# cmeraki/audiotoken

Hardware: AMD Instinct MI355X
Metric: audio-sec tokenized / wall-sec (acoustic + semantic_m) (higher is better)
Workload: dtype f32 (linear layers: two fp16 pieces per operand, three MFMA products, fp32 accumulate)

## Files before the change

### audiotoken_amd/_cabi.py

```python
from __future__ import annotations

import ctypes as C
import os
from pathlib import Path

import numpy as np

_LIB_PATH = Path(__file__).resolve().parent / "lib" / "libaudiotoken_hip.so"
_lib = None


class HipLibraryError(RuntimeError):
    pass


class SegmentDesc(C.Structure):
    _fields_ = [("pcm", C.c_void_p), ("table", C.c_void_p), ("chunk_off", C.c_int64), ("chunk_len", C.c_int32), ("out_start", C.c_int32),
                ("valid_len", C.c_int32), ("fmt", C.c_int32), ("scale", C.c_float), ("o", C.c_int32), ("n", C.c_int32), ("width", C.c_int32),
                ("chunk_out_len", C.c_int32)]


PCM_S16, PCM_S32, PCM_F32, PCM_U8 = 0, 1, 2, 3


# ... 114 lines not shown
    "at_hubert_profile_read": (C.c_int, [C.c_void_p, C.c_char_p, C.c_size_t, C.POINTER(C.c_float), C.POINTER(C.c_int), C.c_int]),
    "at_encodec_range_sites": (C.c_int, [C.c_char_p, C.c_size_t]),
    "at_encodec_range_report": (C.c_int, [C.c_void_p, C.POINTER(C.c_float), C.c_int]),
    "at_w2vbert_range_sites": (C.c_int, [C.c_char_p, C.c_size_t]),
    "at_w2vbert_range_report": (C.c_int, [C.c_void_p, C.POINTER(C.c_float), C.c_int]),
    "at_w2vbert_site_scales": (C.c_int, [C.c_void_p, C.POINTER(C.c_float), C.c_int]),
    "at_hubert_site_scales": (C.c_int, [C.c_void_p, C.POINTER(C.c_float), C.c_int]),
    "at_w2vbert_layer_status": (C.c_int, [C.c_void_p, C.POINTER(C.c_int32), C.c_int]),
    "at_hubert_layer_status": (C.c_int, [C.c_void_p, C.POINTER(C.c_int32), C.c_int]),
    "at_hubert_range_sites": (C.c_int, [C.c_char_p, C.c_size_t]),
    "at_hubert_range_report": (C.c_int, [C.c_void_p, C.POINTER(C.c_float), C.c_int]),
    "at_segments_from_pcm": (C.c_int, [C.c_void_p, C.c_int, C.c_int, C.c_float, C.c_void_p, C.c_void_p, C.c_void_p]),
    "at_clock_stamp": (C.c_int, [C.c_void_p, C.c_void_p]),
    "at_resample_rows": (C.c_int, [C.c_void_p, C.c_int, C.c_void_p, C.c_void_p]),
    "at_resample_rows_check": (C.c_int, [C.c_void_p, C.c_int]),
    "at_segments_zmuv_workspace_bytes": (C.c_size_t, [C.c_int, C.c_int]),
    "at_segments_from_pcm_zmuv": (C.c_int, [C.c_void_p, C.c_int, C.c_int, C.c_int, C.c_float, C.c_float, C.c_void_p, C.c_void_p, C.c_void_p, C.c_size_t, C.c_void_p]),
    "at_pcm_peaks": (C.c_int, [C.c_void_p, C.c_void_p, C.c_int, C.c_int64, C.c_void_p, C.c_void_p]),
    "at_pcm_pack": (C.c_int, [C.c_void_p, C.c_void_p, C.c_int, C.c_int64, C.c_float, C.c_void_p, C.c_void_p, C.c_void_p]),
    "at_flac_encode_workspace_bytes": (C.c_size_t, [C.c_int]),
    "at_flac_encode_rows": (C.c_int, [C.c_void_p, C.c_void_p, C.c_int, C.c_int, C.c_float, C.c_void_p, C.c_void_p, C.c_int64, C.c_void_p, C.c_void_p, C.c_size_t,
                                      C.c_void_p]),
    "at_flac_encode_pcm16": (C.c_int64, [C.c_void_p, C.c_int64, C.c_int, C.c_void_p, C.c_int64, C.c_void_p, C.c_int64, C.c_int64]),
    "at_flac_write_frames": (C.c_int64, [C.c_void_p, C.c_int, C.c_void_p, C.c_int64, C.c_int, C.c_void_p, C.c_int, C.c_void_p, C.c_int64, C.c_void_p]),
    "at_flac_streaminfo": (C.c_int, [C.c_int, C.c_int, C.c_int, C.c_int, C.c_int, C.c_int64, C.c_void_p]),
    "at_flac_info": (C.c_int, [C.c_void_p, C.c_size_t, C.POINTER(C.c_int), C.POINTER(C.c_int), C.POINTER(C.c_int), C.POINTER(C.c_int64), C.c_void_p]),
    "at_flac_decode": (C.c_int64, [C.c_void_p, C.c_size_t, C.c_void_p, C.c_int64]),
    "at_op_layernorm": (C.c_int, [C.c_void_p, C.c_void_p, C.c_void_p, C.c_void_p, C.c_void_p, C.c_int64, C.c_int, C.c_void_p]),
    "at_op_relpos_attention": (C.c_int, [C.c_void_p, C.c_void_p, C.c_void_p, C.c_void_p, C.c_int, C.c_int, C.c_void_p]),
    "at_op_relpos_attention_kvp": (C.c_int, [C.c_void_p, C.c_void_p, C.c_void_p, C.c_float, C.c_void_p, C.c_int, C.c_int, C.c_int, C.c_int, C.c_void_p, C.c_size_t,
                                             C.c_void_p, C.c_void_p]),
    "at_op_dwconv_ln_swish": (C.c_int, [C.c_void_p, C.c_void_p, C.c_void_p, C.c_void_p, C.c_void_p, C.c_int, C.c_int, C.c_void_p]),
    "at_op_dwconv_stream": (C.c_int, [C.c_void_p, C.c_void_p, C.c_void_p, C.c_void_p, C.c_void_p, C.c_int, C.c_int, C.c_void_p]),
    "at_op_vq_argmax": (C.c_int, [C.c_void_p, C.c_void_p, C.c_void_p, C.c_void_p, C.c_int64, C.c_int, C.c_int, C.c_void_p]),
    "at_op_vq_argmax_refined": (C.c_int, [C.c_void_p, C.c_void_p, C.c_void_p, C.c_void_p, C.c_void_p, C.c_int64, C.c_int, C.c_int, C.c_void_p]),
    "at_kmeans_device_bytes": (C.c_size_t, [C.c_int64, C.c_int, C.c_int]),
    "at_kmeans_create": (C.c_void_p, [C.c_int, C.c_int64, C.c_int, C.c_int]),
    "at_kmeans_destroy": (None, [C.c_void_p]),
    "at_kmeans_set_option": (C.c_int, [C.c_void_p, C.c_char_p, C.c_int]),
    "at_kmeans_get_option": (C.c_int, [C.c_void_p, C.c_char_p]),
    "at_kmeans_set_data": (C.c_int, [C.c_void_p, C.c_void_p, C.c_float, C.c_void_p]),
    "at_kmeans_plusplus": (C.c_int, [C.c_void_p, C.c_void_p, C.c_int, C.c_void_p, C.c_void_p, C.c_void_p]),
    "at_kmeans_assign": (C.c_int, [C.c_void_p, C.c_void_p, C.c_float, C.c_void_p, C.c_void_p, C.c_void_p]),
    "at_kmeans_update": (C.c_int, [C.c_void_p, C.c_void_p, C.c_void_p, C.c_void_p, C.c_void_p, C.c_void_p, C.c_void_p, C.c_void_p]),
    "at_kmeans_layernorm": (C.c_int, [C.c_void_p, C.c_void_p, C.c_int64, C.c_int, C.c_int, C.c_void_p, C.c_size_t, C.c_void_p]),
    "at_kmeans_row_d2": (C.c_int, [C.c_void_p, C.c_void_p, C.c_void_p]),
    "at_kmeans_relocations": (C.c_int, [C.c_void_p, C.c_void_p, C.c_void_p]),
    "at_op_gemm": (C.c_int, [C.POINTER(GemmDesc), C.c_void_p]),
    "at_op_gemm_dual": (C.c_int, [C.POINTER(GemmDesc), C.c_void_p, C.c_int64, C.c_int, C.c_int, C.c_void_p]),
    "at_op_gemm_route": (C.c_int, [C.POINTER(GemmDesc), C.c_void_p, C.c_int64, C.c_int, C.c_int, C.POINTER(C.c_int32)]),
    "at_op_attention_f32": (C.c_int, [C.c_void_p, C.c_void_p, C.c_void_p, C.c_void_p, C.c_int, C.c_int, C.c_int, C.c_void_p]),
    "at_required_tensors": (C.c_int, [C.c_char_p, C.c_int, C.c_int, C.c_char_p, C.c_size_t]),
    "at_op_gemm_split": (C.c_int, [C.c_void_p, C.c_void_p, C.c_void_p, C.c_void_p, C.c_int, C.c_int, C.c_int, C.c_int, C.c_float, C.c_int,
                                   C.c_void_p, C.c_size_t, C.c_void_p, C.c_void_p]),
    "at_op_conv_split": (C.c_int, [C.c_void_p, C.c_void_p, C.c_void_p, C.c_void_p, C.c_int, C.c_int, C.c_int, C.c_int, C.c_int, C.c_int, C.c_float,
                                  C.c_void_p, C.c_size_t, C.c_void_p, C.c_void_p]),
    "at_op_rvq_encode_split": (C.c_int, [C.c_void_p, C.c_int64, C.c_int, C.c_void_p, C.c_void_p, C.c_int, C.c_void_p, C.c_int, C.c_float,
                                        C.c_void_p, C.c_size_t, C.c_void_p, C.c_void_p]),
    "at_op_rvq_encode": (C.c_int, [C.c_void_p, C.c_int64, C.c_int, C.c_void_p, C.c_void_p, C.c_int, C.c_void_p, C.c_void_p]),
    "at_gpt_create": (C.c_void_p, [C.c_int]),
    "at_gpt_set_tensor": (C.c_int, [C.c_void_p, C.c_char_p, C.c_void_p, C.POINTER(C.c_int64), C.c_int]),
    "at_gpt_finalize": (C.c_int, [C.c_void_p]),
    "at_gpt_destroy": (None, [C.c_void_p]),
    "at_gpt_num_layers": (C.c_int, [C.c_void_p]),
    "at_gpt_vocab": (C.c_int, [C.c_void_p]),
    "at_gpt_block_size": (C.c_int, [C.c_void_p]),
# ... 186 lines not shown
```

### audiotoken_amd/csrc/dwconv_stream.hip

```cpp
#include "at_common.h"
#include "w2vbert_kernels.h"
#include "split_scheme.h"

#include <type_traits>

namespace at {

namespace {

constexpr int DS_K = 31;
constexpr int DS_RB = 8;
constexpr int DS_WIN = DS_RB + DS_K - 1;
constexpr int DS_C = 1024;

__device__ __forceinline__ float ds_quad_xor1(float x) { return __builtin_bit_cast(float, __builtin_amdgcn_mov_dpp(__builtin_bit_cast(int, x), 0xB1, 0xF, 0xF, true)); }
__device__ __forceinline__ float ds_quad_xor2(float x) { return __builtin_bit_cast(float, __builtin_amdgcn_mov_dpp(__builtin_bit_cast(int, x), 0x4E, 0xF, 0xF, true)); }

template <bool SECOND>
__device__ __forceinline__ void ds_reduce(float (&v)[DS_RB], float (*sq)[256], float (*stat)[4], int c, int lane) {
#pragma unroll
    for (int i = 0; i < DS_RB; ++i) {
        float p = v[i] + ds_quad_xor1(v[i]);
        p = p + ds_quad_xor2(p);
        if ((lane & 3) == 0) sq[i][c >> 2] = p;
    }
    __syncthreads();
    const int wave = c >> 6;
    if (wave < DS_RB) {
        float t[4];
#pragma unroll
        for (int grp = 0; grp < 4; ++grp) t[grp] = sq[wave][grp * 64 + lane];
#pragma unroll
        for (int off = 32; off >= 1; off >>= 1)
#pragma unroll
            for (int grp = 0; grp < 4; ++grp) t[grp] += __shfl_xor(t[grp], off);
        if (lane == 0) {
            const float total = (t[0] + t[1]) + (t[2] + t[3]);
            if (!SECOND) {
                stat[wave][0] = total * (1.0f / 1024.0f);
            } else {
                const float vr = total * (1.0f / 1024.0f);
                const float rstd = 1.0f / sqrtf(vr + 1e-5f);
                stat[wave][1] = rstd;
                stat[wave][2] = -rstd * stat[wave][0];
            }
        }
    }
    __syncthreads();
}

}

template <class SC>
__global__ __launch_bounds__(1024, 1) void dwconv_stream_kernel(const float* __restrict__ g, const float* __restrict__ w ,
                                                                const float* __restrict__ gamma, const float* __restrict__ beta,
                                                                float* __restrict__ out, int T, int seg_len, void* __restrict__ pieces, long long rows_pad,
                                                                float scale, int* __restrict__ status) {
    __shared__ float sq[DS_RB][256];
    __shared__ __attribute__((aligned(16))) float stat[DS_RB][4];
    __shared__ __attribute__((aligned(16))) float otile[DS_RB][DS_C + 4];
    const int c = threadIdx.x, lane = c & 63;
    const int b = blockIdx.y;
    const int t_begin = blockIdx.x * seg_len;
    if (t_begin >= T) return;
    const int t_end = t_begin + seg_len < T ? t_begin + seg_len : T;
    const long long base = (long long)b * T;
    const float* gc = g + base * DS_C + c;

    float wt[DS_K];
#pragma unroll
    for (int j = 0; j < DS_K; ++j) wt[j] = w[j * DS_C + c];
    float xw[DS_WIN];
#pragma unroll
    for (int k = 0; k < DS_K - 1; ++k) {
        const int t = t_begin - (DS_K - 1) + k;
        xw[k] = t >= 0 ? gc[(long long)t * DS_C] : 0.f;
    }
    float pre[DS_RB];
    auto prefetch = [&](int tb) {
#pragma unroll
        for (int i = 0; i < DS_RB; ++i) {
            int t = tb + i;
            t = t < T ? t : T - 1;
            pre[i] = gc[(long long)t * DS_C];
        }
    };
    prefetch(t_begin);
    RangeMax over;
    (void)over;
    for (int tb = t_begin; tb < t_end; tb += DS_RB) {
#pragma unroll
        for (int i = 0; i < DS_RB; ++i) xw[DS_K - 1 + i] = pre[i];
        if (tb + DS_RB < t_end) prefetch(tb + DS_RB);
        float acc[DS_RB];
#pragma unroll
        for (int i = 0; i < DS_RB; ++i) {
            float a = 0.f;
#pragma unroll
            for (int tap = 0; tap < DS_K; ++tap) a = __builtin_fmaf(wt[tap], xw[i + tap], a);
            acc[i] = a;
        }
        float term[DS_RB];
#pragma unroll
        for (int i = 0; i < DS_RB; ++i) term[i] = acc[i];
        ds_reduce<false>(term, sq, stat, c, lane);
#pragma unroll
        for (int i = 0; i < DS_RB; ++i) {
            const float d = acc[i] - stat[i][0];
            const float m = __fmul_rn(d, d);
            const float f = __builtin_fmaf(d, d, ds_quad_xor1(m));
            term[i] = (lane & 1) ? 0.f : f;
        }
        ds_reduce<true>(term, sq, stat, c, lane);
        const float* gp = gamma;
        const float* bp = beta;
        asm volatile("" : "+s"(gp), "+s"(bp));
        const float gm = gp[c], bt = bp[c];
#pragma unroll
        for (int i = 0; i < DS_RB; ++i) {
            const int t = tb + i;
            const float o = swishf_(fmaf(fmaf(acc[i], stat[i][1], stat[i][2]), gm, bt));
            if constexpr (std::is_void<SC>::value) {
                if (t < t_end) out[(base + t) * DS_C + c] = o;
            } else {
                otile[i][c] = o;
            }
        }
        if constexpr (!std::is_void<SC>::value) {
            __syncthreads();
#pragma unroll
            for (int j = 0; j < 2; ++j) {
                const int e = c + 1024 * j, i = (e >> 2) & (DS_RB - 1), qd = ((e >> 5) << 2) | (e & 3);
                const int t = tb + i;
                if (t < t_end) {
                    const f4 o = *reinterpret_cast<const f4*>(&otile[i][qd * 4]);
                    over |= store_pieces4<SC>(reinterpret_cast<typename SC::T*>(pieces), rows_pad * DS_C, rows_pad, base + t, qd * 4, o, scale);
                }
            }
        }
#pragma unroll
        for (int k = 0; k < DS_K - 1; ++k) xw[k] = xw[k + DS_RB];
    }
    if constexpr (!std::is_void<SC>::value)
        if constexpr (SC::RANGE_CHECK)
            range_publish(status, status ? status + 1 : nullptr, over);
}

int launch_dwconv_stream(const float* g, const float* w, const float* gamma, const float* beta, float* out, int B, int T, hipStream_t stream,
                         const SplitOut& split) {
    __bf16* const pieces = split.pieces;
    const long long rows_pad = split.rows_pad;
    const int scheme = split.scheme;
    const float scale = split.scale;
    int* const status = split.status;
    const int cus = device_cus();
    int nseg = (cus + B - 1) / B;
    const int max_seg = (T + DS_RB - 1) / DS_RB;
    nseg = nseg < 1 ? 1 : (nseg > max_seg ? max_seg : nseg);
    const int seg_len = ((T + nseg - 1) / nseg + DS_RB - 1) / DS_RB * DS_RB;
    dim3 grid((T + seg_len - 1) / seg_len, B);
    if (pieces && scheme == XB_SCHEME_F16X2)
        hipLaunchKernelGGL((dwconv_stream_kernel<SchemeF16x2>), grid, dim3(1024), 0, stream, g, w, gamma, beta, out, T, seg_len, (void*)pieces, rows_pad, scale, status);
    else if (pieces)
        hipLaunchKernelGGL((dwconv_stream_kernel<SchemeBf16x3>), grid, dim3(1024), 0, stream, g, w, gamma, beta, out, T, seg_len, (void*)pieces, rows_pad, scale, status);
    else
        hipLaunchKernelGGL((dwconv_stream_kernel<void>), grid, dim3(1024), 0, stream, g, w, gamma, beta, out, T, seg_len, nullptr, 0LL, 1.0f, nullptr);
    AT_CHECK_HIP(hipGetLastError());
    return 0;
}

}
```

### audiotoken_amd/csrc/semantic_ops.hip

```cpp
#include "../../include/audiotoken_hip.h"
#include "gemm_bf16x3.h"
#include "w2vbert_kernels.h"

using namespace at;

extern "C" {

int at_op_layernorm(const float* x, const float* gamma, const float* beta, const float* row_mask, float* y, int64_t rows, int D,
                    at_stream_t stream) {
    AT_REQUIRE(x && y, "null pointer");
    return launch_layernorm(x, gamma, beta, row_mask, y, rows, D, (hipStream_t)stream);
}

int at_op_relpos_attention(const float* qkv, const float* attn_mask, const float* dist_emb80, float* ctx, int B, int T,
                           at_stream_t stream) {
    AT_REQUIRE(qkv && attn_mask && dist_emb80 && ctx && B >= 1 && T >= 1, "bad arguments");
    AttnArgs a;
    a.qkv = qkv; a.amask = attn_mask; a.dist_emb = dist_emb80; a.ctx = ctx; a.B = B; a.T = T;
    return launch_relpos_attention(a, (hipStream_t)stream);
}

int at_op_attention_f32(const float* qkv, const float* attn_mask, const float* dist_emb80, float* ctx, int B, int T, int heads, at_stream_t stream) {
    AT_REQUIRE(qkv && attn_mask && ctx && B >= 1 && T >= 1 && heads >= 1 && heads <= 64, "bad arguments");
    AttnArgs a;
// ... 2 lines not shown
}

int at_op_relpos_attention_kvp(const float* qkv, const float* attn_mask, const float* dist_emb80, float dist_max_abs, float* ctx, int B, int T, int heads, int w8,
                               void* kv_workspace, size_t kv_workspace_bytes, int32_t* status_dev, at_stream_t stream) {
    AT_REQUIRE(qkv && attn_mask && ctx && kv_workspace && B >= 1 && T >= 1 && heads >= 1 && heads <= 64, "bad arguments");
    const long long rows = (long long)B * T, rows_pad = (rows + 255) / 256 * 256;
    const int hid = heads * 64;
    const size_t kv_bytes = (size_t)4 * rows_pad * hid * 2, dist_bytes = (size_t)2 * 96 * 64 * 2;
    AT_REQUIRE(kv_workspace_bytes >= kv_bytes + dist_bytes, "kv workspace too small: 4 * ceil256(B * T) * heads * 64 * 2 + 24576 bytes");
    if (int rc = launch_kv_rowmajor_split(qkv, static_cast<__bf16*>(kv_workspace), rows, rows_pad, hid, status_dev, (hipStream_t)stream)) return rc;
    AttnArgs a;
    a.qkv = qkv; a.amask = attn_mask; a.dist_emb = dist_emb80; a.ctx = ctx; a.B = B; a.T = T; a.heads = heads; a.arith = 2;
    a.status = status_dev; a.rows_pad = rows_pad; a.kv_pieces = static_cast<const __bf16*>(kv_workspace); a.w8 = w8;
    if (dist_emb80) {
        __bf16* dist_s = reinterpret_cast<__bf16*>(static_cast<char*>(kv_workspace) + kv_bytes);
        a.dist = SplitW{dist_s, xb_weight_scale(dist_max_abs)};
        if (int rc = launch_dist_split(dist_emb80, dist_s, a.dist.s, (hipStream_t)stream)) return rc;
    }
    return launch_relpos_attention(a, (hipStream_t)stream);
}

int at_op_dwconv_ln_swish(const float* g, const float* w31x1024, const float* gamma, const float* beta, float* out, int B, int T,
                          at_stream_t stream) {
    AT_REQUIRE(g && w31x1024 && gamma && beta && out && B >= 1 && T >= 1, "bad arguments");
    return launch_dwconv_ln_swish(g, w31x1024, gamma, beta, out, B, T, (hipStream_t)stream);
}

int at_op_dwconv_stream(const float* g, const float* w31x1024, const float* gamma, const float* beta, float* out, int B, int T,
                        at_stream_t stream) {
    AT_REQUIRE(g && w31x1024 && gamma && beta && out && B >= 1 && T >= 1, "bad arguments");
    return launch_dwconv_stream(g, w31x1024, gamma, beta, out, B, T, (hipStream_t)stream);
}

int at_op_vq_argmax(const float* x, const float* dots, const float* e2, int16_t* out, int64_t rows, int D, int C, at_stream_t stream) {
    AT_REQUIRE(x && dots && e2 && out && D % 4 == 0 && C % 4 == 0, "bad arguments");
    return launch_vq_argmax(x, dots, e2, out, rows, D, C, (hipStream_t)stream);
}

int at_op_vq_argmax_refined(const float* x, const float* dots, const float* e2, const float* codebook, int16_t* out, int64_t rows, int D, int C, at_stream_t stream) {
    AT_REQUIRE(x && dots && e2 && codebook && out && D % 4 == 0 && C % 4 == 0, "bad arguments");
    return launch_vq_argmax(x, dots, e2, out, rows, D, C, (hipStream_t)stream, nullptr, 0, codebook);
}

}
```

### audiotoken_amd/csrc/w2vbert_kernels.h

```cpp
#pragma once
#include "at_common.h"
#include "gemm_bf16x3.h"

namespace at {

int launch_frame_prep(const float* wav, const float* smask, const float* window, double* frames, float* fmask, int B, int N,
                      int F, hipStream_t stream, int* status = nullptr);
int launch_dft_f64(const double* frames, const double* dft, float* spec, long long M, int N, hipStream_t stream);
int launch_fbank_normalize(const float* logmel, const float* fmask, float* stats, float* feats, float* amask, int B, int F, int Tp,
                           hipStream_t stream);
int launch_layernorm(const float* x, const float* gamma, const float* beta, const float* row_mask, float* y, long long rows, int D,
                     hipStream_t stream);
struct AttnArgs {
    const float* qkv = nullptr;
    const float* amask = nullptr;
    const float* dist_emb = nullptr;
    float* ctx = nullptr;
    int B = 0, T = 0, heads = 16;
    int arith = -1;
    int* status = nullptr;
    piece_t* ctx_pieces = nullptr;
    long long rows_pad = 0;
    const piece_t* kv_pieces = nullptr;
    int w8 = -1;
    SplitW dist;
};
int launch_relpos_attention(const AttnArgs& a, hipStream_t stream);
int launch_relpos_attention_x3(const AttnArgs& a, int scheme, hipStream_t stream);
bool relpos_attention_w8_eligible(int T, int heads, long long rows_pad, long long B, bool relpos);
int launch_relpos_attention_w8(const AttnArgs& a, hipStream_t stream);
int launch_dist_split(const float* dist_emb, __bf16* out, float scale, hipStream_t stream);
int launch_kv_rowmajor_split(const float* qkv, __bf16* out, long long rows, long long rows_pad, int hid, int* status, hipStream_t stream);
int launch_dwconv_ln_swish(const float* g, const float* w, const float* gamma, const float* beta, float* out, int B, int T, hipStream_t stream,
                           const SplitOut& split = {});
int launch_dwconv_stream(const float* g, const float* w, const float* gamma, const float* beta, float* out, int B, int T, hipStream_t stream,
                         const SplitOut& split = {});
int launch_layernorm_split(const float* x, const float* gamma, const float* beta, const float* row_mask, float* y, long long rows, int D, const SplitOut& split,
                           hipStream_t stream);
int launch_layernorm2_split(const float* x, const float* gamma, const float* beta, float* y, const float* gamma2, const float* beta2, long long rows, int D,
                            const SplitOut& split, hipStream_t stream);
int launch_vq_argmax(const float* x, const float* dots, const float* e2, int16_t* out, long long rows, int D, int C,
// ... 4 lines not shown
```

### audiotoken_amd/csrc/w2vbert_kernels.hip

```cpp
#include "gemm_core.h"
#include "w2vbert_kernels.h"
#include "split_scheme.h"
#include <cstdlib>
#include <type_traits>

namespace at {

__global__ __launch_bounds__(256) void frame_prep_kernel(const float* __restrict__ wav, const float* __restrict__ smask,
                                                         const float* __restrict__ window, double* __restrict__ frames,
                                                         float* __restrict__ fmask, int N, int F, long long total_frames, int* __restrict__ status) {
    const int lane = threadIdx.x & 63;
    const long long fid = (long long)blockIdx.x * 4 + (threadIdx.x >> 6);
    if (fid >= total_frames) return;
    const long long b = fid / F;
    const int f = (int)(fid - b * F);
    const float* x = wav + b * N + (long long)f * 160;
    double v[7];
    double sum = 0.0;
    bool all_valid = true;
#pragma unroll
    for (int j = 0; j < 7; ++j) {
        const int n = lane + 64 * j;
        v[j] = n < 400 ? (double)x[n] * 32768.0 : 0.0;
        sum += v[j];
// ... 58 lines not shown
#pragma unroll
            for (int e = 0; e < 4; ++e) As[srow * DFT_LD + sk + e] = m < M ? frames[m * DFT_K + k0 + sk + e] : 0.0;
            const int n = n0 + srow;
#pragma unroll
            for (int e = 0; e < 4; ++e) Bs[srow * DFT_LD + sk + e] = n < N ? dft[(long long)n * DFT_K + k0 + sk + e] : 0.0;
        }
        __syncthreads();
#pragma unroll
        for (int e = 0; e < 4; ++e) {
            const int k = q * 4 + e;
            double a[2], bb[2];
#pragma unroll
            for (int i = 0; i < 2; ++i) a[i] = As[(wm * 32 + i * 16 + r16) * DFT_LD + k];
#pragma unroll
            for (int j = 0; j < 2; ++j) bb[j] = Bs[(wn * 32 + j * 16 + r16) * DFT_LD + k];
#pragma unroll
            for (int i = 0; i < 2; ++i)
#pragma unroll
                for (int j = 0; j < 2; ++j) acc[i][j] = __builtin_amdgcn_mfma_f64_16x16x4f64(a[i], bb[j], acc[i][j], 0, 0, 0);
        }
    }
#pragma unroll
    for (int i = 0; i < 2; ++i)
#pragma unroll
        for (int j = 0; j < 2; ++j)
#pragma unroll
            for (int reg = 0; reg < 4; ++reg) {
                const long long m = m0 + wm * 32 + i * 16 + q + 4 * reg;
                const int n = n0 + wn * 32 + j * 16 + r16;
                if (m < M && n < N) spec[m * N + n] = (float)acc[i][j][reg];
            }
}

int launch_dft_f64(const double* frames, const double* dft, float* spec, long long M, int N, hipStream_t stream) {
    if (M <= 0) return 0;
    dim3 grid((unsigned)((M + 63) / 64), (N + 63) / 64);
    hipLaunchKernelGGL(dft_f64_kernel, grid, dim3(256), 0, stream, frames, dft, spec, M, N);
    AT_CHECK_HIP(hipGetLastError());
    return 0;
}

__global__ __launch_bounds__(320) void fbank_stats_kernel(const float* __restrict__ logmel, const float* __restrict__ fmask,
                                                          float* __restrict__ stats , int F) {
    __shared__ double red[4][80];
    __shared__ float mean_s[80];
    __shared__ double cnt_s;
    const int b = blockIdx.x;
    const int bin = threadIdx.x % 80, grp = threadIdx.x / 80;
    const float* x = logmel + (long long)b * F * 80;
    const float* m = fmask + (long long)b * F;
    double s = 0.0, c = 0.0;
    for (int f = grp; f < F; f += 4) {
        const float mk = m[f];
        s += (double)(x[(long long)f * 80 + bin] * mk);
        c += (double)mk;
    }
    red[grp][bin] = s;
    __syncthreads();
    __shared__ double cred[4];
    if (bin == 0) cred[grp] = c;
    __syncthreads();
    if (threadIdx.x == 0) cnt_s = fmax((cred[0] + cred[1]) + (cred[2] + cred[3]), 1.0);
    __syncthreads();
    if (grp == 0) mean_s[bin] = (float)(((red[0][bin] + red[1][bin]) + (red[2][bin] + red[3][bin])) / cnt_s);
    __syncthreads();
    const float mean = mean_s[bin];
    double v = 0.0;
    for (int f = grp; f < F; f += 4) {
        const float mk = m[f];
        const float d = x[(long long)f * 80 + bin] * mk - mean;
        v += (double)(d * d * mk);
    }
    __syncthreads();
    red[grp][bin] = v;
    __syncthreads();
    if (grp == 0) {
        stats[((long long)b * 2 + 0) * 80 + bin] = mean;
        stats[((long long)b * 2 + 1) * 80 + bin] = (float)(((red[0][bin] + red[1][bin]) + (red[2][bin] + red[3][bin])) / cnt_s);
    }
}

__global__ __launch_bounds__(256) void fbank_stack_kernel(const float* __restrict__ logmel, const float* __restrict__ fmask,
                                                          const float* __restrict__ stats, float* __restrict__ feats,
                                                          float* __restrict__ amask, int F, int Tp, long long total) {
    const long long gid = (long long)blockIdx.x * 256 + threadIdx.x;
    if (gid >= total) return;
    const int c4 = (int)(gid % 40);
    const long long bt = gid / 40;
    const long long b = bt / Tp;
    const int t = (int)(bt - b * Tp);
    const int half = c4 >= 20;
    const int bin = (c4 - half * 20) * 4;
    const int f = 2 * t + half;
    const int Fs = F / 2;
    f4 o = {1.f, 1.f, 1.f, 1.f};
    const bool exists = t < Fs;
    if (exists && fmask[b * F + f] != 0.f) {
        const f4 x = *reinterpret_cast<const f4*>(logmel + (b * F + f) * 80 + bin);
        const f4 mu = *reinterpret_cast<const f4*>(stats + (b * 2 + 0) * 80 + bin);
        const f4 var = *reinterpret_cast<const f4*>(stats + (b * 2 + 1) * 80 + bin);
#pragma unroll
        for (int k = 0; k < 4; ++k) o[k] = (x[k] - mu[k]) / sqrtf(var[k] + 1e-7f);
    }
    *reinterpret_cast<f4*>(feats + bt * 160 + c4 * 4) = o;
    if (c4 == 0) amask[bt] = (exists && fmask[b * F + 2 * t] != 0.f) ? 1.0f : 0.0f;
}

int launch_fbank_normalize(const float* logmel, const float* fmask, float* stats, float* feats, float* amask, int B, int F, int Tp,
                           hipStream_t stream) {
    hipLaunchKernelGGL(fbank_stats_kernel, dim3(B), dim3(320), 0, stream, logmel, fmask, stats, F);
    AT_CHECK_HIP(hipGetLastError());
    const long long total = (long long)B * Tp * 40;
    hipLaunchKernelGGL(fbank_stack_kernel, dim3((unsigned)((total + 255) / 256)), dim3(256), 0, stream, logmel, fmask, stats,
                       feats, amask, F, Tp, total);
    AT_CHECK_HIP(hipGetLastError());
    return 0;
}

template <int MAXV>
__global__ __launch_bounds__(256) void layernorm_kernel(const float* __restrict__ x, const float* __restrict__ gamma,
                                                        const float* __restrict__ beta, const float* __restrict__ row_mask,
                                                        float* __restrict__ y, long long rows, int D) {
    const int lane = threadIdx.x & 63;
    const long long row = (long long)blockIdx.x * 4 + (threadIdx.x >> 6);
    if (row >= rows) return;
    const int nv = D >> 2;
    const f4* xr = reinterpret_cast<const f4*>(x + row * D);
    f4 v[MAXV];
    float s = 0.f;
#pragma unroll
    for (int j = 0; j < MAXV; ++j) {
        const int c = lane + 64 * j;
        v[j] = c < nv ? xr[c] : f4{0.f, 0.f, 0.f, 0.f};
        s += (v[j].x + v[j].y) + (v[j].z + v[j].w);
    }
#pragma unroll
    for (int off = 32; off >= 1; off >>= 1) s += __shfl_xor(s, off);
    const float mean = s / (float)D;
    float q = 0.f;
#pragma unroll
    for (int j = 0; j < MAXV; ++j) {
        const int c = lane + 64 * j;
        if (c < nv) {
            const f4 d = v[j] - mean;
// ... 656 lines not shown
```

### include/audiotoken_hip.h

```cpp
#ifndef AUDIOTOKEN_HIP_H
#define AUDIOTOKEN_HIP_H

#include <stddef.h>
#include <stdint.h>

#ifdef __cplusplus
extern "C" {
#endif

typedef void* at_stream_t;

int at_version(void);
const char* at_last_error(void);

typedef struct at_encodec at_encodec_t;

at_encodec_t* at_encodec_create(int device_id);

int at_encodec_set_tensor(at_encodec_t* h, const char* name, const float* host_data, const int64_t* shape, int ndim);

int at_encodec_finalize(at_encodec_t* h, int with_decoder);
void at_encodec_destroy(at_encodec_t* h);
int at_encodec_num_codebooks(const at_encodec_t* h);

// ... 181 lines not shown
int at_op_gemm_dual(const at_gemm_desc* d, const float* X2, int64_t x2_bstride, int ld2, int K1, at_stream_t stream);
int at_op_gemm_route(const at_gemm_desc* d, const float* X2, int64_t x2_bstride, int ld2, int K1, int32_t* out);

int at_required_tensors(const char* model, int n, int with_extras, char* buf, size_t cap);

int at_op_gemm_split(const float* X, const float* W, const float* bias, float* C, int M, int N, int K, int scheme, float w_max_abs,
                     int kernel, void* workspace, size_t workspace_bytes, int32_t* status_dev, at_stream_t stream);
int at_op_conv_split(const float* X, const float* W, const float* bias, float* C, int B, int L, int Cin, int Cout, int ktaps, int stride,
                     float w_max_abs, void* workspace, size_t workspace_bytes, int32_t* status_dev, at_stream_t stream);
int at_op_rvq_encode(const float* x, int64_t rows, int T, const float* codebooks, const float* e2, int n_q,
                     int16_t* codes, at_stream_t stream);
int at_op_rvq_encode_split(const float* x, int64_t rows, int T, const float* codebooks, const float* e2, int n_q, int16_t* codes, int scheme,
                           float cb_max_abs, void* workspace, size_t workspace_bytes, int32_t* status_dev, at_stream_t stream);

int at_op_hub_conv0(const float* wav, const float* w, const float* gamma, const float* beta, float* out, int B, int N, void* workspace,
                    size_t workspace_bytes, at_stream_t stream);
int at_op_hub_frame_mask(const float* smask, float* fmask, int B, int N, int T, at_stream_t stream);

int at_op_layernorm(const float* x, const float* gamma, const float* beta, const float* row_mask, float* y, int64_t rows, int D,
                    at_stream_t stream);

int at_op_relpos_attention(const float* qkv, const float* attn_mask, const float* dist_emb80, float* ctx, int B, int T,
                           at_stream_t stream);

int at_op_attention_f32(const float* qkv, const float* attn_mask, const float* dist_emb80, float* ctx, int B, int T, int heads, at_stream_t stream);

int at_op_relpos_attention_kvp(const float* qkv, const float* attn_mask, const float* dist_emb80, float dist_max_abs, float* ctx, int B, int T, int heads, int w8,
                               void* kv_workspace, size_t kv_workspace_bytes, int32_t* status_dev, at_stream_t stream);

int at_op_dwconv_ln_swish(const float* g, const float* w31x1024, const float* gamma, const float* beta, float* out, int B, int T,
                          at_stream_t stream);
int at_op_dwconv_stream(const float* g, const float* w31x1024, const float* gamma, const float* beta, float* out, int B, int T,
                        at_stream_t stream);

int at_op_vq_argmax(const float* x, const float* dots, const float* e2, int16_t* out, int64_t rows, int D, int C, at_stream_t stream);
int at_op_vq_argmax_refined(const float* x, const float* dots, const float* e2, const float* codebook, int16_t* out, int64_t rows, int D, int C, at_stream_t stream);

typedef struct at_kmeans at_kmeans_t;

size_t at_kmeans_device_bytes(int64_t N, int D, int K);
at_kmeans_t* at_kmeans_create(int device, int64_t N, int D, int K);
void at_kmeans_destroy(at_kmeans_t* h);
int at_kmeans_set_option(at_kmeans_t* h, const char* name, int value);
int at_kmeans_get_option(const at_kmeans_t* h, const char* name);
int at_kmeans_set_data(at_kmeans_t* h, const float* X, float x_max_abs, at_stream_t stream);
int at_kmeans_plusplus(at_kmeans_t* h, const double* uniforms, int trials, float* C_out, int64_t* picked_rows, at_stream_t stream);
int at_kmeans_assign(at_kmeans_t* h, const float* C, float c_max_abs, int16_t* labels, int32_t* status_dev, at_stream_t stream);
int at_kmeans_update(at_kmeans_t* h, const int16_t* labels, const int16_t* prev_labels, const float* C_old, float* C_new, int32_t* counts,
                     double* stats_dev, at_stream_t stream);
int at_kmeans_layernorm(const float* x, float* y, int64_t rows, int D, int split_kernel, void* workspace, size_t workspace_bytes, at_stream_t stream);
int at_kmeans_row_d2(const at_kmeans_t* h, double* out, at_stream_t stream);
int at_kmeans_relocations(const at_kmeans_t* h, int32_t* out, at_stream_t stream);

typedef struct at_gpt at_gpt_t;
at_gpt_t* at_gpt_create(int device_id);
int at_gpt_set_tensor(at_gpt_t* h, const char* name, const float* host_data, const int64_t* shape, int ndim);
int at_gpt_finalize(at_gpt_t* h);
void at_gpt_destroy(at_gpt_t* h);
int at_gpt_num_layers(const at_gpt_t* h);
int at_gpt_vocab(const at_gpt_t* h);
int at_gpt_block_size(const at_gpt_t* h);
size_t at_gpt_state_bytes(const at_gpt_t* h, int B, int max_len);
#define AT_GPT_FINISH_STOP 1
#define AT_GPT_FINISH_MAX_NEW 2
#define AT_GPT_FINISH_BLOCK 3
int at_gpt_generate(at_gpt_t* h, const int32_t* prompts_dev, int prompt_stride, const int32_t* prompt_len, int B, int max_new, float temperature, int top_k,
// ... 100 lines not shown
```

Measured before the change: 15650.

## Add async LDS ring to dwconv stream and new DFT and fbank-stats kernels

The depthwise conv stream kernel now prefetches input rows into a three-slot dynamic-LDS ring with global_load_lds DMA, two blocks ahead, and uses counted vmcnt waits in place of a register prefetch. A new single-pass f64 DFT kernel keeps the frame operands in registers and streams DFT matrix rows through a register ring, one 64-thread block per 32 frames. A new fbank stats kernel double-buffers its loads. Both new kernels are the default variants and are exposed through new C API ops. The hand-counted waits assume a fixed DMA count, and the smaller DFT blocks may reduce occupancy.

```diff
diff --git a/audiotoken_amd/_cabi.py b/audiotoken_amd/_cabi.py
--- a/audiotoken_amd/_cabi.py
+++ b/audiotoken_amd/_cabi.py
@@ -170,6 +170,8 @@
                                              C.c_void_p, C.c_void_p]),
     "at_op_dwconv_ln_swish": (C.c_int, [C.c_void_p, C.c_void_p, C.c_void_p, C.c_void_p, C.c_void_p, C.c_int, C.c_int, C.c_void_p]),
     "at_op_dwconv_stream": (C.c_int, [C.c_void_p, C.c_void_p, C.c_void_p, C.c_void_p, C.c_void_p, C.c_int, C.c_int, C.c_void_p]),
+    "at_op_dft_f64": (C.c_int, [C.c_void_p, C.c_void_p, C.c_void_p, C.c_int64, C.c_int, C.c_int, C.c_void_p]),
+    "at_op_fbank_stats": (C.c_int, [C.c_void_p, C.c_void_p, C.c_void_p, C.c_int, C.c_int, C.c_int, C.c_void_p]),
     "at_op_vq_argmax": (C.c_int, [C.c_void_p, C.c_void_p, C.c_void_p, C.c_void_p, C.c_int64, C.c_int, C.c_int, C.c_void_p]),
     "at_op_vq_argmax_refined": (C.c_int, [C.c_void_p, C.c_void_p, C.c_void_p, C.c_void_p, C.c_void_p, C.c_int64, C.c_int, C.c_int, C.c_void_p]),
     "at_kmeans_device_bytes": (C.c_size_t, [C.c_int64, C.c_int, C.c_int]),
diff --git a/audiotoken_amd/csrc/dwconv_stream.hip b/audiotoken_amd/csrc/dwconv_stream.hip
--- a/audiotoken_amd/csrc/dwconv_stream.hip
+++ b/audiotoken_amd/csrc/dwconv_stream.hip
@@ -12,19 +12,29 @@
 constexpr int DS_RB = 8;
 constexpr int DS_WIN = DS_RB + DS_K - 1;
 constexpr int DS_C = 1024;
+constexpr int DS_SLOTS = 3;
+constexpr int DS_AHEAD = 2;
+constexpr int DS_DMA_PER_WAVE = DS_RB * DS_C * 4 / 1024 / 16;
+constexpr size_t DS_RING_BYTES = (size_t)DS_SLOTS * DS_RB * DS_C * sizeof(float);
+static_assert(DS_AHEAD == 2 && DS_SLOTS == 3 && DS_DMA_PER_WAVE == 2, "the counted waits below are written for two blocks of two DMA instructions in flight");
+
+typedef __attribute__((address_space(3))) void ds_lds_void;
+typedef const __attribute__((address_space(1))) void ds_glb_void;
+
+__device__ __forceinline__ void ds_barrier() { asm volatile("s_waitcnt lgkmcnt(0)\n\ts_barrier" ::: "memory"); }
 
 __device__ __forceinline__ float ds_quad_xor1(float x) { return __builtin_bit_cast(float, __builtin_amdgcn_mov_dpp(__builtin_bit_cast(int, x), 0xB1, 0xF, 0xF, true)); }
 __device__ __forceinline__ float ds_quad_xor2(float x) { return __builtin_bit_cast(float, __builtin_amdgcn_mov_dpp(__builtin_bit_cast(int, x), 0x4E, 0xF, 0xF, true)); }
 
 template <bool SECOND>
-__device__ __forceinline__ void ds_reduce(float (&v)[DS_RB], float (*sq)[256], float (*stat)[4], int c, int lane) {
+__device__ __forceinline__ void ds_reduce(float (&v)[DS_RB], float (*sq)[256], float (*stat)[4], int c, int lane, bool more = false) {
 #pragma unroll
     for (int i = 0; i < DS_RB; ++i) {
         float p = v[i] + ds_quad_xor1(v[i]);
         p = p + ds_quad_xor2(p);
         if ((lane & 3) == 0) sq[i][c >> 2] = p;
     }
-    __syncthreads();
+    ds_barrier();
     const int wave = c >> 6;
     if (wave < DS_RB) {
         float t[4];
@@ -46,7 +56,11 @@
             }
         }
     }
-    __syncthreads();
+    if (SECOND) {
+        if (more) asm volatile("s_waitcnt vmcnt(2)" ::: "memory");
+        else asm volatile("s_waitcnt vmcnt(0)" ::: "memory");
+    }
+    ds_barrier();
 }
 
 }
@@ -59,6 +73,8 @@
     __shared__ float sq[DS_RB][256];
     __shared__ __attribute__((aligned(16))) float stat[DS_RB][4];
     __shared__ __attribute__((aligned(16))) float otile[DS_RB][DS_C + 4];
+    extern __shared__ __attribute__((aligned(16))) unsigned char ds_ring_raw[];
+    float* ring = reinterpret_cast<float*>(ds_ring_raw);
     const int c = threadIdx.x, lane = c & 63;
     const int b = blockIdx.y;
     const int t_begin = blockIdx.x * seg_len;
@@ -66,32 +82,45 @@
     const int t_end = t_begin + seg_len < T ? t_begin + seg_len : T;
     const long long base = (long long)b * T;
     const float* gc = g + base * DS_C + c;
+    const int wave = __builtin_amdgcn_readfirstlane(c >> 6);
+    const int drow = wave >> 1, dcol = (wave & 1) * 512;
+    const float* gq = g + base * DS_C + dcol + lane * 4;
+    auto issue = [&](int tb, int slot) {
+        int t = tb + drow;
+        t = t < T ? t : T - 1;
+        const float* src = gq + (long long)t * DS_C;
+        float* dst = ring + (slot * DS_RB + drow) * DS_C + dcol;
+#pragma unroll
+        for (int j = 0; j < DS_DMA_PER_WAVE; ++j)
+            __builtin_amdgcn_global_load_lds((ds_glb_void*)(src + j * 256), (ds_lds_void*)(dst + j * 256), 16, 0, 0);
+    };
+    issue(t_begin, 0);
+    if (t_begin + DS_RB < t_end) issue(t_begin + DS_RB, 1);
 
     float wt[DS_K];
 #pragma unroll
     for (int j = 0; j < DS_K; ++j) wt[j] = w[j * DS_C + c];
+    const float gm = gamma[c], bt = beta[c];
     float xw[DS_WIN];
 #pragma unroll
     for (int k = 0; k < DS_K - 1; ++k) {
         const int t = t_begin - (DS_K - 1) + k;
         xw[k] = t >= 0 ? gc[(long long)t * DS_C] : 0.f;
     }
-    float pre[DS_RB];
-    auto prefetch = [&](int tb) {
-#pragma unroll
-        for (int i = 0; i < DS_RB; ++i) {
-            int t = tb + i;
-            t = t < T ? t : T - 1;
-            pre[i] = gc[(long long)t * DS_C];
-        }
-    };
-    prefetch(t_begin);
+    asm volatile("s_waitcnt vmcnt(0)" ::: "memory");
+    ds_barrier();
     RangeMax over;
     (void)over;
+    int slot = 0;
     for (int tb = t_begin; tb < t_end; tb += DS_RB) {
-#pragma unroll
-        for (int i = 0; i < DS_RB; ++i) xw[DS_K - 1 + i] = pre[i];
-        if (tb + DS_RB < t_end) prefetch(tb + DS_RB);
+        {
+            const float* rs = ring + slot * (DS_RB * DS_C) + c;
+#pragma unroll
+            for (int i = 0; i < DS_RB; ++i) xw[DS_K - 1 + i] = rs[i * DS_C];
+        }
+        const bool more = tb + DS_AHEAD * DS_RB < t_end;
+        if (more) issue(tb + DS_AHEAD * DS_RB, slot == 0 ? DS_SLOTS - 1 : slot - 1);
+        slot = slot == DS_SLOTS - 1 ? 0 : slot + 1;
         float acc[DS_RB];
 #pragma unroll
         for (int i = 0; i < DS_RB; ++i) {
@@ -111,11 +140,7 @@
             const float f = __builtin_fmaf(d, d, ds_quad_xor1(m));
             term[i] = (lane & 1) ? 0.f : f;
         }
-        ds_reduce<true>(term, sq, stat, c, lane);
-        const float* gp = gamma;
-        const float* bp = beta;
-        asm volatile("" : "+s"(gp), "+s"(bp));
-        const float gm = gp[c], bt = bp[c];
+        ds_reduce<true>(term, sq, stat, c, lane, more);
 #pragma unroll
         for (int i = 0; i < DS_RB; ++i) {
             const int t = tb + i;
@@ -127,7 +152,7 @@
             }
         }
         if constexpr (!std::is_void<SC>::value) {
-            __syncthreads();
+            ds_barrier();
 #pragma unroll
             for (int j = 0; j < 2; ++j) {
                 const int e = c + 1024 * j, i = (e >> 2) & (DS_RB - 1), qd = ((e >> 5) << 2) | (e & 3);
@@ -159,12 +184,17 @@
     nseg = nseg < 1 ? 1 : (nseg > max_seg ? max_seg : nseg);
     const int seg_len = ((T + nseg - 1) / nseg + DS_RB - 1) / DS_RB * DS_RB;
     dim3 grid((T + seg_len - 1) / seg_len, B);
-    if (pieces && scheme == XB_SCHEME_F16X2)
-        hipLaunchKernelGGL((dwconv_stream_kernel<SchemeF16x2>), grid, dim3(1024), 0, stream, g, w, gamma, beta, out, T, seg_len, (void*)pieces, rows_pad, scale, status);
-    else if (pieces)
-        hipLaunchKernelGGL((dwconv_stream_kernel<SchemeBf16x3>), grid, dim3(1024), 0, stream, g, w, gamma, beta, out, T, seg_len, (void*)pieces, rows_pad, scale, status);
-    else
-        hipLaunchKernelGGL((dwconv_stream_kernel<void>), grid, dim3(1024), 0, stream, g, w, gamma, beta, out, T, seg_len, nullptr, 0LL, 1.0f, nullptr);
+    auto launch = [&](auto kernel, LdsAttrFlags& lds_set, void* pc, long long rp, float sc, int* st) -> int {
+        if (int rc = set_max_dynamic_lds(lds_set, kernel, DS_RING_BYTES)) return rc;
+        hipLaunchKernelGGL(kernel, grid, dim3(1024), DS_RING_BYTES, stream, g, w, gamma, beta, out, T, seg_len, pc, rp, sc, st);
+        return 0;
+    };
+    static LdsAttrFlags set_f16, set_bf16, set_f32;
+    int rc;
+    if (pieces && scheme == XB_SCHEME_F16X2) rc = launch(dwconv_stream_kernel<SchemeF16x2>, set_f16, (void*)pieces, rows_pad, scale, status);
+    else if (pieces) rc = launch(dwconv_stream_kernel<SchemeBf16x3>, set_bf16, (void*)pieces, rows_pad, scale, status);
+    else rc = launch(dwconv_stream_kernel<void>, set_f32, nullptr, 0LL, 1.0f, nullptr);
+    if (rc) return rc;
     AT_CHECK_HIP(hipGetLastError());
     return 0;
 }
diff --git a/audiotoken_amd/csrc/semantic_ops.hip b/audiotoken_amd/csrc/semantic_ops.hip
--- a/audiotoken_amd/csrc/semantic_ops.hip
+++ b/audiotoken_amd/csrc/semantic_ops.hip
@@ -58,6 +58,16 @@
     return launch_dwconv_stream(g, w31x1024, gamma, beta, out, B, T, (hipStream_t)stream);
 }
 
+int at_op_dft_f64(const double* frames, const double* dft, float* spec, int64_t M, int N, int variant, at_stream_t stream) {
+    AT_REQUIRE(frames && dft && spec && M >= 0 && N >= 1 && (variant == 0 || variant == 1), "bad arguments");
+    return launch_dft_f64(frames, dft, spec, M, N, (hipStream_t)stream, variant);
+}
+
+int at_op_fbank_stats(const float* logmel, const float* fmask, float* stats, int B, int F, int variant, at_stream_t stream) {
+    AT_REQUIRE(logmel && fmask && stats && B >= 1 && F >= 1 && (variant == 0 || variant == 1), "bad arguments");
+    return launch_fbank_stats(logmel, fmask, stats, B, F, (hipStream_t)stream, variant);
+}
+
 int at_op_vq_argmax(const float* x, const float* dots, const float* e2, int16_t* out, int64_t rows, int D, int C, at_stream_t stream) {
     AT_REQUIRE(x && dots && e2 && out && D % 4 == 0 && C % 4 == 0, "bad arguments");
     return launch_vq_argmax(x, dots, e2, out, rows, D, C, (hipStream_t)stream);
diff --git a/audiotoken_amd/csrc/w2vbert_kernels.h b/audiotoken_amd/csrc/w2vbert_kernels.h
--- a/audiotoken_amd/csrc/w2vbert_kernels.h
+++ b/audiotoken_amd/csrc/w2vbert_kernels.h
@@ -6,7 +6,8 @@
 
 int launch_frame_prep(const float* wav, const float* smask, const float* window, double* frames, float* fmask, int B, int N,
                       int F, hipStream_t stream, int* status = nullptr);
-int launch_dft_f64(const double* frames, const double* dft, float* spec, long long M, int N, hipStream_t stream);
+int launch_dft_f64(const double* frames, const double* dft, float* spec, long long M, int N, hipStream_t stream, int variant = 1);
+int launch_fbank_stats(const float* logmel, const float* fmask, float* stats, int B, int F, hipStream_t stream, int variant = 1);
 int launch_fbank_normalize(const float* logmel, const float* fmask, float* stats, float* feats, float* amask, int B, int F, int Tp,
                            hipStream_t stream);
 int launch_layernorm(const float* x, const float* gamma, const float* beta, const float* row_mask, float* y, long long rows, int D,
diff --git a/audiotoken_amd/csrc/w2vbert_kernels.hip b/audiotoken_amd/csrc/w2vbert_kernels.hip
--- a/audiotoken_amd/csrc/w2vbert_kernels.hip
+++ b/audiotoken_amd/csrc/w2vbert_kernels.hip
@@ -114,10 +114,72 @@
             }
 }
 
-int launch_dft_f64(const double* frames, const double* dft, float* spec, long long M, int N, hipStream_t stream) {
+constexpr int DFT_FR = 32;
+constexpr int DFT_RING = 5;
+static_assert((DFT_K / DFT_BK) % DFT_RING == 0, "static ring indices need the ring to divide the k-blocks of a column block");
+
+__global__ __launch_bounds__(64) void dft_f64_once_kernel(const double* __restrict__ frames, const double* __restrict__ dft,
+                                                          float* __restrict__ spec, long long M, int N) {
+    constexpr int NKB = DFT_K / DFT_BK;
+    const int lane = threadIdx.x;
+    const int r16 = lane & 15, q = lane >> 4;
+    const long long m0 = (long long)blockIdx.x * DFT_FR;
+    d4 a[2][NKB];
+#pragma unroll
+    for (int i = 0; i < 2; ++i) {
+        const long long m = m0 + i * 16 + r16 < M ? m0 + i * 16 + r16 : M - 1;
+        const double* fr = frames + m * DFT_K + q * 4;
+#pragma unroll
+        for (int kb = 0; kb < NKB; ++kb) a[i][kb] = *reinterpret_cast<const d4*>(fr + kb * DFT_BK);
+    }
+    const int ncb = (N + 15) / 16;
+    auto load_b = [&](int cb, int kb) -> d4 {
+        const int n = min(cb * 16 + r16, N - 1);
+        return *reinterpret_cast<const d4*>(dft + (long long)n * DFT_K + kb * DFT_BK + q * 4);
+    };
+    __builtin_amdgcn_s_waitcnt(0x0F70);
+    d4 ring[DFT_RING];
+#pragma unroll
+    for (int j = 0; j < DFT_RING; ++j) ring[j] = load_b(0, j);
+    auto run = [&](auto full_tag, int cb0, int cb1) {
+        constexpr bool FULL = decltype(full_tag)::value;
+        for (int cb = cb0; cb < cb1; ++cb) {
+            d4 acc[2];
+            acc[0] = d4{0., 0., 0., 0.};
+            acc[1] = d4{0., 0., 0., 0.};
+#pragma unroll
+            for (int kb = 0; kb < NKB; ++kb) {
+                const d4 b = ring[kb % DFT_RING];
+                if (kb + DFT_RING < NKB) ring[kb % DFT_RING] = load_b(cb, kb + DFT_RING);
+                else ring[kb % DFT_RING] = load_b(min(cb + 1, ncb - 1), kb + DFT_RING - NKB);
+#pragma unroll
+                for (int e = 0; e < 4; ++e)
+#pragma unroll
+                    for (int i = 0; i < 2; ++i) acc[i] = __builtin_amdgcn_mfma_f64_16x16x4f64(a[i][kb][e], b[e], acc[i], 0, 0, 0);
+                __builtin_amdgcn_sched_barrier(0);
+            }
+            const int n = cb * 16 + r16;
+            float* so = spec + (m0 + q) * N + n;
+#pragma unroll
+            for (int i = 0; i < 2; ++i)
+#pragma unroll
+                for (int reg = 0; reg < 4; ++reg)
+                    if (FULL || (m0 + i * 16 + q + 4 * reg < M && n < N)) so[(long long)(i * 16 + 4 * reg) * N] = (float)acc[i][reg];
+        }
+    };
+    const int nfull = m0 + DFT_FR <= M ? N / 16 : 0;
+    run(std::true_type{}, 0, nfull);
+    run(std::false_type{}, nfull, ncb);
+}
+
+int launch_dft_f64(const double* frames, const double* dft, float* spec, long long M, int N, hipStream_t stream, int variant) {
     if (M <= 0) return 0;
-    dim3 grid((unsigned)((M + 63) / 64), (N + 63) / 64);
-    hipLaunchKernelGGL(dft_f64_kernel, grid, dim3(256), 0, stream, frames, dft, spec, M, N);
+    if (variant == 0) {
+        dim3 grid((unsigned)((M + 63) / 64), (N + 63) / 64);
+        hipLaunchKernelGGL(dft_f64_kernel, grid, dim3(256), 0, stream, frames, dft, spec, M, N);
+    } else {
+        hipLaunchKernelGGL(dft_f64_once_kernel, dim3((unsigned)((M + DFT_FR - 1) / DFT_FR)), dim3(64), 0, stream, frames, dft, spec, M, N);
+    }
     AT_CHECK_HIP(hipGetLastError());
     return 0;
 }
@@ -160,6 +222,88 @@
         stats[((long long)b * 2 + 0) * 80 + bin] = mean;
         stats[((long long)b * 2 + 1) * 80 + bin] = (float)(((red[0][bin] + red[1][bin]) + (red[2][bin] + red[3][bin])) / cnt_s);
     }
+}
+
+constexpr int FB_BLK = 16;
+__global__ __launch_bounds__(320) void fbank_stats_ahead_kernel(const float* __restrict__ logmel, const float* __restrict__ fmask,
+                                                                float* __restrict__ stats , int F) {
+    __shared__ double red[4][80];
+    __shared__ float mean_s[80];
+    __shared__ double cnt_s;
+    __shared__ double cred[4];
+    const int b = blockIdx.x;
+    const int bin = threadIdx.x % 80, grp = threadIdx.x / 80;
+    const float* x = logmel + (long long)b * F * 80;
+    const float* m = fmask + (long long)b * F;
+    auto fetch = [&](int f0, float (&xv)[FB_BLK], float (&mv)[FB_BLK]) {
+#pragma unroll
+        for (int j = 0; j < FB_BLK; ++j) {
+            const int f = f0 + 4 * j;
+            if (f < F) {
+                mv[j] = m[f];
+                xv[j] = x[(long long)f * 80 + bin];
+            }
+        }
+    };
+    auto walk = [&](auto add) {
+        float xa[FB_BLK], ma[FB_BLK], xb[FB_BLK], mb[FB_BLK];
+        int f0 = grp;
+        if (f0 >= F) return;
+        fetch(f0, xa, ma);
+        for (;;) {
+            fetch(f0 + 4 * FB_BLK, xb, mb);
+            add(f0, xa, ma);
+            f0 += 4 * FB_BLK;
+            if (f0 >= F) break;
+            fetch(f0 + 4 * FB_BLK, xa, ma);
+            add(f0, xb, mb);
+            f0 += 4 * FB_BLK;
+            if (f0 >= F) break;
+        }
+    };
+    double s = 0.0, c = 0.0;
+    walk([&](int f0, const float (&xv)[FB_BLK], const float (&mv)[FB_BLK]) {
+#pragma unroll
+        for (int j = 0; j < FB_BLK; ++j)
+            if (f0 + 4 * j < F) {
+                const float mk = mv[j];
+                s += (double)(xv[j] * mk);
+                c += (double)mk;
+            }
+    });
+    red[grp][bin] = s;
+    __syncthreads();
+    if (bin == 0) cred[grp] = c;
+    __syncthreads();
+    if (threadIdx.x == 0) cnt_s = fmax((cred[0] + cred[1]) + (cred[2] + cred[3]), 1.0);
+    __syncthreads();
+    if (grp == 0) mean_s[bin] = (float)(((red[0][bin] + red[1][bin]) + (red[2][bin] + red[3][bin])) / cnt_s);
+    __syncthreads();
+    const float mean = mean_s[bin];
+    double v = 0.0;
+    walk([&](int f0, const float (&xv)[FB_BLK], const float (&mv)[FB_BLK]) {
+#pragma unroll
+        for (int j = 0; j < FB_BLK; ++j)
+            if (f0 + 4 * j < F) {
+                const float mk = mv[j];
+                const float d = xv[j] * mk - mean;
+                v += (double)(d * d * mk);
+            }
+    });
+    __syncthreads();
+    red[grp][bin] = v;
+    __syncthreads();
+    if (grp == 0) {
+        stats[((long long)b * 2 + 0) * 80 + bin] = mean;
+        stats[((long long)b * 2 + 1) * 80 + bin] = (float)(((red[0][bin] + red[1][bin]) + (red[2][bin] + red[3][bin])) / cnt_s);
+    }
+}
+
+int launch_fbank_stats(const float* logmel, const float* fmask, float* stats, int B, int F, hipStream_t stream, int variant) {
+    if (variant == 0) hipLaunchKernelGGL(fbank_stats_kernel, dim3(B), dim3(320), 0, stream, logmel, fmask, stats, F);
+    else hipLaunchKernelGGL(fbank_stats_ahead_kernel, dim3(B), dim3(320), 0, stream, logmel, fmask, stats, F);
+    AT_CHECK_HIP(hipGetLastError());
+    return 0;
 }
 
 __global__ __launch_bounds__(256) void fbank_stack_kernel(const float* __restrict__ logmel, const float* __restrict__ fmask,
@@ -190,8 +334,7 @@
 
 int launch_fbank_normalize(const float* logmel, const float* fmask, float* stats, float* feats, float* amask, int B, int F, int Tp,
                            hipStream_t stream) {
-    hipLaunchKernelGGL(fbank_stats_kernel, dim3(B), dim3(320), 0, stream, logmel, fmask, stats, F);
-    AT_CHECK_HIP(hipGetLastError());
+    if (int rc = launch_fbank_stats(logmel, fmask, stats, B, F, stream)) return rc;
     const long long total = (long long)B * Tp * 40;
     hipLaunchKernelGGL(fbank_stack_kernel, dim3((unsigned)((total + 255) / 256)), dim3(256), 0, stream, logmel, fmask, stats,
                        feats, amask, F, Tp, total);
diff --git a/include/audiotoken_hip.h b/include/audiotoken_hip.h
--- a/include/audiotoken_hip.h
+++ b/include/audiotoken_hip.h
@@ -237,6 +237,9 @@
                           at_stream_t stream);
 int at_op_dwconv_stream(const float* g, const float* w31x1024, const float* gamma, const float* beta, float* out, int B, int T,
                         at_stream_t stream);
+
+int at_op_dft_f64(const double* frames, const double* dft, float* spec, int64_t M, int N, int variant, at_stream_t stream);
+int at_op_fbank_stats(const float* logmel, const float* fmask, float* stats, int B, int F, int variant, at_stream_t stream);
 
 int at_op_vq_argmax(const float* x, const float* dots, const float* e2, int16_t* out, int64_t rows, int D, int C, at_stream_t stream);
 int at_op_vq_argmax_refined(const float* x, const float* dots, const float* e2, const float* codebook, int16_t* out, int64_t rows, int D, int C, at_stream_t stream);
```

New measurement: 15740, median of 6. No clear change (+0.6%).
